# Illumina/Pisces

Measured on AMD Instinct MI355X. Metric: candidate loci/s at 500x depth, higher is better.
Workload: dtype int32 counts + f64 likelihoods; 1 GPU; BASELINE config 2: synthetic 100000 loci x 500x amplicon pileup, SNV-only, gVCF, per GPU per step; device-resident packed tuples; depth=500, ring_batches=6, tile_loci=56, parallelism=interval-shard x1

## Files before the change

### pisces_amd/csrc/device_math.hip.h

```cpp
#pragma once
#include <hip/hip_runtime.h>
#include <stdint.h>

#include "../../include/pisces_hip.h"
#include "poisson_core.h"

namespace pisces {

struct DeviceParams {
    int32_t min_bq, noise_level, max_vq, min_vq, vq_filter, min_cov, low_depth_filter;
    int32_t min_gq, max_gq, low_gq_filter, sb_model, filter_single_strand, include_ref, emit_zero_cov;
    int32_t rmxn_max_len, rmxn_min_rep;
    float min_freq, vf_filter, gt_min_freq, target_lod, nocall_thr, rmxn_freq_limit;
    double sb_threshold;
    double err_q;
    double err_sb;
    double ln10;
    unsigned long long* totals;
    const double* q_to_p_lut;
    int32_t q_to_p_n;
    const double* gq_tail;
    int32_t gq_tail_a, gq_tail_cov;
    int32_t refs_only;
    int32_t variants_only;
// ... 405 lines not shown
        reverseBias = (rev.var_gt_zero * fwd.false_pos) / overall.var_gt_zero;
        if (overall.var_gt_zero == 0) {
            forwardBias = 1;
            reverseBias = 1;
        }
    }
    double score = forwardBias > reverseBias ? forwardBias : reverseBias;
    cov_both = (cf > 0) && (cr > 0);
    var_both = (sf > 0) && (sr > 0);
    if (!cov_both) score = 0;
    bias_score = score;
    acceptable = score < P.sb_threshold;
    return ok0 && ok1 && ok2;
}

__device__ __forceinline__ int32_t somatic_gq_index(int32_t genotype, int32_t cov, int32_t support, const DeviceParams& P)
{
    if (cov == 0 || !((genotype == PISCES_GT_HOM_REF) || (genotype == PISCES_GT_HOM_ALT))) return -1;
    const float nonAlleleObservationsF = (1.0f - frequency_f(support, cov)) * (float)cov;
    const float expectedNonAllelObservationsF = P.target_lod * (float)cov;
    if (nonAlleleObservationsF >= expectedNonAllelObservationsF) return -1;
    const int ai = (int)((double)nonAlleleObservationsF + 1.0);
    if (ai >= 1 && ai < P.gq_tail_a && cov < P.gq_tail_cov) return ai * P.gq_tail_cov + cov;
    return -1;
}
__device__ __forceinline__ bool somatic_gq_try(int32_t genotype, int32_t variantQ, int32_t cov, int32_t support, const DeviceParams& P,
                                               int32_t gq_index, int32_t gq_cap_value , int32_t& gq)
{
    const bool noCall = (genotype == PISCES_GT_ALT12_LIKE_NOCALL || genotype == PISCES_GT_ALT_LIKE_NOCALL || genotype == PISCES_GT_REF_LIKE_NOCALL);
    if ((cov == 0) || noCall) { gq = P.min_gq; return true; }
    if ((genotype == PISCES_GT_HOM_REF) || (genotype == PISCES_GT_HOM_ALT)) {
        if (gq_index >= 0 && variantQ == P.max_vq && P.gq_cap) { gq = gq_cap_value; return true; }
        const float nonAlleleObservationsF = (1.0f - frequency_f(support, cov)) * (float)cov;
        const float expectedNonAllelObservationsF = P.target_lod * (float)cov;
        if (nonAlleleObservationsF >= expectedNonAllelObservationsF) { gq = P.min_gq; return true; }
        return false;
    }
    double qScore = fmin((double)P.max_gq, (double)variantQ);
    qScore = fmax(qScore, (double)P.min_gq);
    gq = (int32_t)rint(qScore);
    return true;
}

struct AlleleTables {
    int32_t vq;
    double sb[3];
    int32_t gq_cap;
    int32_t gq_idx;
    uint32_t have;
};
__device__ __forceinline__ bool tables_complete(const DeviceParams& P) { return P.vq_tab && P.sb_tab && P.sb0_tab && P.gq_cap; }

__device__ __forceinline__ AlleleTables request_allele_tables(bool isRef, int32_t support, int32_t total, int32_t refsup, const int32_t cov[3],
                                                              const int32_t sup[3], const DeviceParams& P)
{
    AlleleTables t;
    const uint32_t tab_cov = (uint32_t)P.tab_cov;
    const bool vq_in = support > 0 && total > 0 && support < P.vq_tab_k && total < P.tab_cov;
    const int16_t vq_v = P.vq_tab[vq_in ? (uint32_t)support * tab_cov + (uint32_t)total : 0u];
    const int s2 = sup[2] / 2, c2 = cov[2] / 2;
    const int ss[3] = {sup[0] + sup[1] + sup[2], sup[0] + s2, sup[1] + s2};
    const int cc[3] = {cov[0] + cov[1] + cov[2], cov[0] + c2, cov[1] + c2};
    double sb_v[3];
    uint32_t have = vq_in ? 1u : 0u;
#pragma unroll
    for (int w = 0; w < 3; w++) {
        const bool zero = ss[w] == 0;
        const bool in = zero ? (P.sb_model != PISCES_SB_POISSON && cc[w] >= 0 && cc[w] < P.tab_cov)
                             : (ss[w] > 0 && ss[w] < P.sb_tab_k && cc[w] >= 0 && cc[w] < P.tab_cov);
        const double* base = zero ? P.sb0_tab : P.sb_tab;
        const uint32_t idx = in ? (zero ? (uint32_t)cc[w] : (uint32_t)ss[w] * tab_cov + (uint32_t)cc[w]) : 0u;
        sb_v[w] = base[idx];
        have |= in ? (2u << w) : 0u;
    }
    t.gq_idx = somatic_gq_index(somatic_genotype(isRef, total, support, refsup, P), total, support, P);
    const int16_t gq_v = P.gq_cap[t.gq_idx >= 0 ? t.gq_idx : 0];
    t.vq = vq_v;
    t.sb[0] = sb_v[0]; t.sb[1] = sb_v[1]; t.sb[2] = sb_v[2];
    t.gq_cap = gq_v;
    t.have = have;
    return t;
}

__device__ __forceinline__ bool poisson_qscore_try(int32_t callCount, int32_t coverage, const DeviceParams& P, const AlleleTables& t, int32_t& vq)
{
    if ((callCount <= 0) || (coverage <= 0)) { vq = 0; return true; }
    if (t.have & 1u) { vq = t.vq; return true; }
    const double lambda = P.err_q * coverage;
    if (P.max_vq <= 110 && callCount >= 3 && (double)callCount >= 2.0 * lambda) {
        const double km1 = callCount - 1;
        const double need = ((double)P.max_vq + 1.0) * 0.23025850929940458 + 1e-3;
        if (km1 * (ln_ratio_lower_bound(km1, lambda) - 1.0) >= need) { vq = P.max_vq; return true; }
    }
    return false;
}

__device__ __forceinline__ bool sb_stats_try(int32_t support, int32_t coverage, const DeviceParams& P, bool have, double value, SbStats& st)
{
    st.support = (double)support;
    st.coverage = (double)coverage;
    if (support == 0) {
        if (P.sb_model == PISCES_SB_POISSON) {
            st.false_pos = 1;
            st.var_gt_zero = 0;
            return true;
        }
        if (!have) return false;
        st.var_gt_zero = value;
        st.false_pos = 1 - st.var_gt_zero;
        return true;
    }
    if (have) {
        st.var_gt_zero = value;
    } else {
        const double a = (double)support, x = (double)coverage * P.err_sb;
        if (!(x > 0.0 && 2.0 * x <= a && a * (ln_ratio_lower_bound(a, x) - 1.0) + x > 51.0)) return false;
        st.var_gt_zero = 1.0;
    }
    st.false_pos = fmax(0.0, 1 - st.var_gt_zero);
    return true;
}

__device__ __forceinline__ bool strand_bias_try(const int32_t cov[3], const int32_t sup[3], const DeviceParams& P, const AlleleTables& t,
                                                double& bias_score, int& acceptable, int& var_both, int& cov_both)
{
    const int s2 = sup[2] / 2, c2 = cov[2] / 2;
    const int sf = sup[0] + s2, sr = sup[1] + s2, cf = cov[0] + c2, cr = cov[1] + c2;
    SbStats overall, fwd, rev;
    const bool ok0 = sb_stats_try(sup[0] + sup[1] + sup[2], cov[0] + cov[1] + cov[2], P, (t.have & 2u) != 0, t.sb[0], overall);
    const bool ok1 = sb_stats_try(sf, cf, P, (t.have & 4u) != 0, t.sb[1], fwd);
    const bool ok2 = sb_stats_try(sr, cr, P, (t.have & 8u) != 0, t.sb[2], rev);
    double forwardBias = 0.0, reverseBias = 0.0;
    if (!(fwd.false_pos == 0.0 && rev.false_pos == 0.0 && overall.var_gt_zero > 0.0)) {
        forwardBias = (fwd.var_gt_zero * rev.false_pos) / overall.var_gt_zero;
        reverseBias = (rev.var_gt_zero * fwd.false_pos) / overall.var_gt_zero;
        if (overall.var_gt_zero == 0) {
            forwardBias = 1;
            reverseBias = 1;
        }
    }
    double score = forwardBias > reverseBias ? forwardBias : reverseBias;
    cov_both = (cf > 0) && (cr > 0);
    var_both = (sf > 0) && (sr > 0);
    if (!cov_both) score = 0;
    bias_score = score;
    acceptable = score < P.sb_threshold;
    return ok0 && ok1 && ok2;
}

__device__ __noinline__ int32_t poisson_qscore_out_of_line(int32_t callCount, int32_t coverage, double err, int32_t max_vq, double ln10)
{
    const QParams q = {max_vq, ln10};
    return poisson_qscore_core(callCount, coverage, err, q);
}
struct SbPair { double var_gt_zero, false_pos; };
__device__ __noinline__ SbPair sb_stats_out_of_line(double support, double coverage, double noiseFreq, int model)
{
    const SbStats st = sb_create_stats<false>(support, coverage, noiseFreq, 0.0, model);
    SbPair p = {st.var_gt_zero, st.false_pos};
    return p;
}
__device__ inline SbResult strand_bias_out_of_line(const int32_t cov[3], const int32_t sup[3], const DeviceParams& P)
{
    const int s2 = sup[2] / 2, c2 = cov[2] / 2;
    SbStats st[3];
#pragma unroll 1
// ... 66 lines not shown
```

### pisces_amd/csrc/kernels.hip.h

```cpp
#pragma once
#include <hip/hip_runtime.h>
#include <stdint.h>

#include "device_math.hip.h"
#include "genotype_core.h"

namespace pisces {

constexpr int kBlock = 256;
constexpr int kTile = 64;
constexpr int kFolded = 18;
constexpr int kUnroll = 8;
constexpr int kSlotsPerTile = 4 * kTile;
#ifndef PISCES_TOTAL_SHARDS
#define PISCES_TOTAL_SHARDS 64
#endif
constexpr int kTotalShards = PISCES_TOTAL_SHARDS;
constexpr int kTotalStride = 16;
constexpr int kRefMargin = 32;
constexpr int kRefWin = kTile + 2 * kRefMargin;
constexpr int kWaveRows = 32;
constexpr int kWaveRow = kTile;
constexpr int kWaveRegion = kWaveRows * kWaveRow;
constexpr int kQLutLds = 128;

typedef uint32_t u32x4 __attribute__((ext_vector_type(4)));

__device__ __forceinline__ int allele_of_rank(int k) { return k == 1 ? 2 : (k == 2 ? 1 : k); }
__device__ __forceinline__ int rank_of_allele(int a) { return a == 1 ? 2 : (a == 2 ? 1 : a); }

__device__ __forceinline__ int allele_type_of_base(uint8_t c)
{
    return c == 'A' ? 0 : c == 'G' ? 1 : c == 'C' ? 2 : c == 'T' ? 3 : 4;
}

__device__ __forceinline__ void accumulate_folded(int* hist, uint32_t t, uint32_t n_loci, uint32_t min_bq)
{
    uint32_t locus = PISCES_TUPLE_LOCUS(t);
    uint32_t dir = PISCES_TUPLE_DIR(t);
    uint32_t allele = PISCES_TUPLE_ALLELE(t);
    uint32_t qual = PISCES_TUPLE_QUAL(t);
    if (allele < 4u && qual < min_bq) allele = 4u;
    if (locus < n_loci && dir < 3u && allele < 6u) atomicAdd(&hist[(allele * 3u + dir) * kTile + locus], 1);
}

__device__ __forceinline__ void accumulate_wave(int* hist, uint32_t t, uint32_t min_bq_shifted)
{
    const uint32_t region = (t < min_bq_shifted) ? (uint32_t)(kWaveRegion * sizeof(int)) : 0u;
    const uint32_t off = (t & 0x1FFCu) | region;
    atomicAdd(reinterpret_cast<int*>(reinterpret_cast<char*>(hist) + off), 1);
}

template <typename Op>
__device__ __forceinline__ void stream_tuples(const uint32_t* __restrict__ tuples, int64_t begin, int64_t end, Op op)
{
    const int tid = threadIdx.x;
    int64_t abegin = (begin + 3) & ~(int64_t)3;
    int64_t aend = end & ~(int64_t)3;
    if (abegin > aend) { abegin = end; aend = end; }
    for (int64_t i = begin + tid; i < abegin; i += kBlock) op(tuples[i]);
    const u32x4* __restrict__ p4 = reinterpret_cast<const u32x4*>(tuples + abegin);
    const int64_t n4 = (aend - abegin) >> 2;
    for (int64_t i = tid; i < n4; i += (int64_t)kBlock * kUnroll) {
        u32x4 v[kUnroll];
#pragma unroll
        for (int u = 0; u < kUnroll; u++) {
            int64_t j = i + (int64_t)u * kBlock;
            v[u] = j < n4 ? __builtin_nontemporal_load(&p4[j]) : (u32x4){~0u, ~0u, ~0u, ~0u};
        }
#pragma unroll
        for (int u = 0; u < kUnroll; u++) {
            op(v[u].x); op(v[u].y); op(v[u].z); op(v[u].w);
        }
    }
    for (int64_t i = aend + tid; i < end; i += kBlock) op(tuples[i]);
}

__device__ __forceinline__ void copy_record(PiscesCalledAllele* dst, const PiscesCalledAllele* src)
{
    const unsigned long long sb = (unsigned long long)__double_as_longlong(src->strand_bias_score);
    uint4* dp = reinterpret_cast<uint4*>(dst);
    dp[0] = make_uint4((uint32_t)src->position, (uint32_t)src->total_coverage, (uint32_t)src->allele_support, (uint32_t)src->reference_support);
    dp[1] = make_uint4((uint32_t)src->num_no_calls, (uint32_t)src->coverage_by_dir[0], (uint32_t)src->coverage_by_dir[1], (uint32_t)src->coverage_by_dir[2]);
    dp[2] = make_uint4((uint32_t)src->support_by_dir[0], (uint32_t)src->support_by_dir[1], (uint32_t)src->support_by_dir[2], (uint32_t)src->variant_qscore);
    dp[3] = make_uint4((uint32_t)sb, (uint32_t)(sb >> 32), (uint32_t)(uint16_t)src->genotype_qscore | ((uint32_t)(uint16_t)src->noise_level << 16), (uint32_t)src->filter_bits | ((uint32_t)src->info << 16));
}

struct PointCounts {
    int cov[3], sup[3];
    int total, nocalls, refsup, support;
};

struct HistBlock {
    static __device__ __forceinline__ int idx(int a, int d, int l) { return (a * 3 + d) * kTile + l; }
};
struct HistWave {
    static __device__ __forceinline__ int idx(int a, int d, int l) { return (a * 4 + d) * kWaveRow + (int)PISCES_TUPLE_COLUMN(l, d); }
};

struct HistLinear {
    static __device__ __forceinline__ int idx(int a, int d, int l) { return (a * 4 + d) * kWaveRow + l; }
};

struct LocusCounts { int h[6][3]; };

template <typename H = HistBlock>
__device__ __forceinline__ LocusCounts load_counts(const int* hist, int l)
{
    LocusCounts lc;
#pragma unroll
    for (int k = 0; k < kFolded; k++) lc.h[k / 3][k % 3] = hist[H::idx(k / 3, k % 3, l)];
    return lc;
}

template <typename HistWave = pisces::HistWave>
__device__ __forceinline__ LocusCounts load_counts_wave(const int* hist, int l)
// ... 351 lines not shown
            v[u] = __builtin_nontemporal_load(&p4[j]);
        }
    };
    auto consume = [&](const u32x4* v) {
#pragma unroll
        for (int u = 0; u < kWaveUnroll; u++) { op(v[u].x); op(v[u].y); op(v[u].z); op(v[u].w); }
    };
    const bool streams = (uint32_t)wid < nb;
    if (NW == 2) {
        if (streams) load(cur, (uint32_t)__builtin_amdgcn_readfirstlane(wid));
        __builtin_amdgcn_sched_barrier(0);
        pre();
    } else {
        pre();
        if (streams) load(cur, (uint32_t)__builtin_amdgcn_readfirstlane(wid));
    }
    for (int64_t i = begin + tid; i < abegin; i += 64 * NW) op(tuples[i]);
    if (streams) {
        uint32_t b = (uint32_t)__builtin_amdgcn_readfirstlane(wid);
        const uint32_t m = (nb - b + NW - 1) / NW;
        for (uint32_t p = (m - 1) / 2; p > 0; p--) {
            load(nxt, b + NW);
            __builtin_amdgcn_sched_barrier(0);
            consume(cur);
            __builtin_amdgcn_sched_barrier(0);
            load(cur, b + 2 * NW);
            __builtin_amdgcn_sched_barrier(0);
            consume(nxt);
            __builtin_amdgcn_sched_barrier(0);
            b += 2 * NW;
        }
        if (((m - 1) & 1u) != 0) {
            load(nxt, b + NW);
            __builtin_amdgcn_sched_barrier(0);
            consume(cur);
            __builtin_amdgcn_sched_barrier(0);
#pragma unroll
            for (int u = 0; u < kWaveUnroll; u++) cur[u] = nxt[u];
            b += NW;
        }
        if (b == nb - 1 && (n4 % kBatch)) {
#pragma unroll
            for (int u = 0; u < kWaveUnroll; u++)
                if (b * kBatch + (uint32_t)u * 64u + (uint32_t)lane >= n4) cur[u] = (u32x4){~0u, ~0u, ~0u, ~0u};
        }
        consume(cur);
    }
    for (int64_t i = aend + tid; i < end; i += 64 * NW) op(tuples[i]);
}

__device__ __forceinline__ void wave_lds_sync()
{
    __builtin_amdgcn_fence(__ATOMIC_SEQ_CST, "workgroup");
    __builtin_amdgcn_wave_barrier();
}

template <typename H = HistWave>
__device__ __forceinline__ uint32_t slow_alleles(const int* hist, const uint8_t* s_refwin, uint32_t slow, int l, int pos, int rt, int ref_rank,
                                                 const uint8_t* __restrict__ ref, int64_t win_lo, int64_t win_hi, PiscesCalledAllele* slots,
                                                 const DeviceParams& P)
{
    uint32_t called = 0;
    const int ref_a = (rt < 4) ? rt : PISCES_ALLELE_N;
#pragma unroll 1
    for (int k = 0; k < 5; k++) {
        if (!((slow >> k) & 1u)) continue;
        const bool isRef = k == 4;
        const int a = isRef ? ref_a : allele_of_rank(k);
        const LocusCounts lc = load_counts_wave<H>(hist, l);
        const PointCounts c = point_counts_of(lc, a, isRef, rt, 0);
        int vq = 0;
        if (c.support > 0 && c.total != 0) vq = poisson_qscore_out_of_line(c.support, c.total, P.err_q, P.max_vq, P.ln10);
        if (!isRef && vq < P.min_vq) continue;
        SbResult sb = {0.0, 0, 0, 0};
        if (c.support > 0) sb = strand_bias_out_of_line(c.cov, c.sup, P);
        PiscesCalledAllele r;
        (void)finish_allele<false>(c, pos, a, isRef, rt, vq, sb, ref, win_lo, win_hi, P, r, s_refwin, kRefMargin + l);
        copy_record(&slots[isRef ? ref_rank : k], &r);
        if (!isRef) called |= 1u << k;
    }
    return called;
}

template <int NW, typename H = HistWave>
__device__ __forceinline__ void call_phase_wave(const int* hist, const uint8_t* s_refwin, uint8_t* s_vmask, const PiscesTile& tile, const int t,
                                                const int l, const int wid, const uint8_t* __restrict__ ref, const int32_t ref_start,
                                                const int64_t ref_len, PiscesCalledAllele* __restrict__ records,
                                                PiscesTileResult* __restrict__ tile_results, const DeviceParams& P
#ifdef PISCES_TIMING
                                                , const long long tc0, const long long tc1
#endif
                                                )
{
    const int pos = tile.start_position + l;
    const uint8_t refb = s_refwin[kRefMargin + l];
    const bool in_ref = l < tile.n_loci && refb != 0;
    const int rt = in_ref ? allele_type_of_base(refb) : PISCES_ALLELE_N;
    const int64_t win_lo = (int64_t)ref_start - 1, win_hi = win_lo + ref_len;
    auto slot_of = [&](int k) { return records + ((int64_t)t * kSlotsPerTile + l * 4 + k); };
    const bool dirty = locus_is_dirty(P, pos);
    const LocusCounts lc = load_counts_wave<H>(hist, l);
    const bool ref_wave = wid == 0, var_wave = wid == NW - 1;
    if (P.folded_out && ref_wave && l < tile.n_loci) {
        const unsigned rel = (unsigned)(pos - P.folded_first);
        if (rel < (unsigned)P.folded_n) {
            int32_t* const dst = P.folded_out + (size_t)rel * PISCES_FOLDED_PER_LOCUS;
#pragma unroll
            for (int a = 0; a < 6; a++)
#pragma unroll
                for (int d = 0; d < 3; d++) dst[a * 3 + d] = lc.h[a][d];
        }
    }

    const bool tabs = tables_complete(P);
    auto fast_allele = [&](const PointCounts& c, int a, bool isRef, PiscesCalledAllele& rec) -> bool {
        int vq = 0;
        double sb_score = 0.0;
        int sb_ok = 0, sb_var = 0, sb_cov = 0;
        if (!tabs) return false;
        const AlleleTables tb = request_allele_tables(isRef, c.support, c.total, c.refsup, c.cov, c.sup, P);
        if (c.support > 0 && c.total != 0 && !poisson_qscore_try(c.support, c.total, P, tb, vq)) return false;
        if (!isRef && vq < P.min_vq) return true;
        if (c.support > 0 && !strand_bias_try(c.cov, c.sup, P, tb, sb_score, sb_ok, sb_var, sb_cov)) return false;
        const GqPre g = {tb.gq_idx, tb.gq_cap};
        const SbResult sb = {sb_score, sb_ok, sb_var, sb_cov};
        if (!finish_allele<true>(c, pos, a, isRef, rt, vq, sb, ref, win_lo, win_hi, P, rec, s_refwin, kRefMargin + l, nullptr, &g)) return false;
        return true;
    };
    bool ref_emitted = false;
    int ref_rank = 0;
    uint32_t slow = 0;
    uint32_t vmask = 0;
    const int ref_a = (rt < 4) ? rt : PISCES_ALLELE_N;
    if (ref_wave) {
        const PointCounts c = point_counts_of(lc, ref_a, true, rt, 0);
        if (in_ref && P.include_ref && !P.variants_only && (P.emit_zero_cov || c.total + c.nocalls > 0)) {
            ref_rank = (rt < 4) ? rank_of_allele(rt) : 0;
            ref_emitted = true;
            PiscesCalledAllele rec;
            if (fast_allele(c, ref_a, true, rec)) copy_record(slot_of(ref_rank), &rec);
            else slow |= 16u;
        }
    }
#ifdef PISCES_TIMING
    const long long tcA = wall_clock64();
#endif
    if (var_wave && in_ref && rt < 4 && !P.refs_only && !dirty) {
#pragma unroll 1
        for (int k = 0; k < 4; k++) {
            const int a = allele_of_rank(k);
            if (a == rt) continue;
            const PointCounts c = point_counts_of(lc, a, false, rt, 0);
            if (c.support == 0) continue;
            if (!variant_passes_frequency(c, P)) continue;
            PiscesCalledAllele r;
            r.position = 0;
            if (!fast_allele(c, a, false, r)) { slow |= 1u << k; continue; }
            if (r.position == 0) continue;
            copy_record(slot_of(k), &r);
            vmask |= 1u << k;
        }
    }
    if (__builtin_expect(__ballot(slow != 0) != 0ull, 0))
        vmask |= slow_alleles<H>(hist, s_refwin, slow, l, pos, rt, ref_rank, ref, win_lo, win_hi, records + ((int64_t)t * kSlotsPerTile + l * 4), P);
    if (NW == 2) {
        if (var_wave) s_vmask[l] = (uint8_t)vmask;
        __syncthreads();
        if (!ref_wave) return;
        vmask = s_vmask[l];
    }
#ifdef PISCES_TIMING
    const long long tcB = wall_clock64();
#endif

    const uint32_t valid = vmask ? vmask : (ref_emitted ? (1u << ref_rank) : 0u);
    int n_surv = 0, n_var = 0;
#pragma unroll
    for (int k = 0; k < 4; k++) {
        n_surv += __popcll(__ballot((valid >> k) & 1u));
        n_var += __popcll(__ballot((vmask >> k) & 1u));
    }
    const int n_call_total = n_var + __popcll(__ballot(ref_emitted));
    const int n_loci_called = __popcll(__ballot(valid != 0));
    uint32_t word = valid << ((l & 7) * 4);
    word |= __shfl_xor(word, 1, 64);
    word |= __shfl_xor(word, 2, 64);
    word |= __shfl_xor(word, 4, 64);
    PiscesTileResult* const tile_result = &tile_results[t];
    if ((l & 7) == 0) tile_result->valid[l >> 3] = word;
    if (l == 0) {
        tile_result->record_begin = t * kSlotsPerTile;
        tile_result->n_records = n_surv;
        tile_result->n_candidate_loci = n_loci_called;
        tile_result->n_called = n_call_total;
        if (P.totals) {
            unsigned long long* tt = P.totals + (size_t)(t % kTotalShards) * kTotalStride;
            atomicAdd(&tt[0], (unsigned long long)n_surv);
            atomicAdd(&tt[1], (unsigned long long)n_loci_called);
            atomicAdd(&tt[2], (unsigned long long)n_call_total);
            atomicAdd(&tt[3], 1ull);
        }
#ifdef PISCES_TIMING
        const long long tc2 = wall_clock64();
        tile_result->record_begin = (int)(tc0 & 0x3FFFFFFF);
        tile_result->n_records = (int)(tc1 & 0x3FFFFFFF);
        tile_result->n_candidate_loci = (int)(tc2 & 0x3FFFFFFF);
        tile_result->n_called = (int)__builtin_amdgcn_s_getreg(63492);
        tile_result->valid[0] = __builtin_amdgcn_s_getreg(63508);
        tile_result->valid[1] = 0;
        tile_result->valid[2] = (uint32_t)(tcA - tc1);
        tile_result->valid[3] = (uint32_t)(tcB - tcA);
        tile_result->valid[4] = 0;
        tile_result->valid[5] = (uint32_t)(tc2 - tcB);
#endif
    }
}

template <int NW>
__global__ __launch_bounds__(64 * NW, NW == 1 ? PISCES_WAVE_OCC : PISCES_WAVE2_OCC) void call_tiles_wave_kernel(
    const uint32_t* __restrict__ tuples, const PiscesTile* __restrict__ tiles, int32_t n_tiles,
    const uint8_t* __restrict__ ref, int32_t ref_start, int64_t ref_len, PiscesCalledAllele* __restrict__ records,
    PiscesTileResult* __restrict__ tile_results, DeviceParams P, const DeviceParams* __restrict__ Pd )
{
    __shared__ __attribute__((aligned(16))) int hist[2 * kWaveRegion];
    __shared__ uint8_t s_refwin[kRefWin];
    __shared__ uint8_t s_vmask[kTile];

    const int t = blockIdx.x;
    if (t >= n_tiles) return;
    const int l = threadIdx.x & 63, wid = threadIdx.x >> 6;
    const PiscesTile tile = tiles[t];
#ifdef PISCES_TIMING
    const long long tc0 = wall_clock64();
#endif
    auto setup = [&]() {
        int4* h4 = reinterpret_cast<int4*>(hist);
        for (int i = threadIdx.x; i < 2 * kWaveRegion / 4; i += 64 * NW) h4[i] = make_int4(0, 0, 0, 0);
        for (int i = threadIdx.x; i < kRefWin; i += 64 * NW) {
            const int64_t ri = (int64_t)tile.start_position - kRefMargin + i - ref_start;
            s_refwin[i] = (ri >= 0 && ri < ref_len) ? ref[ri] : (uint8_t)0;
        }
        __syncthreads();
    };

    {
        if (NW == 2) __builtin_amdgcn_s_setprio(3);
        const uint32_t min_bq_shifted = (uint32_t)min(max(P.min_bq, 0), 255) << 24;
        stream_tuples_wave<NW>(tuples, tile.tuple_begin, tile.tuple_end, l, wid, [&](uint32_t v) { accumulate_wave(hist, v, min_bq_shifted); }, setup);
    }
    __syncthreads();
    if (NW == 2) __builtin_amdgcn_s_setprio(0);
#ifdef PISCES_TIMING
    const long long tc1 = wall_clock64();
#endif

    call_phase_wave<NW>(hist, s_refwin, s_vmask, tile, t, l, wid, ref, ref_start, ref_len, records, tile_results, P
#ifdef PISCES_TIMING
                        , tc0, tc1
#endif
                        );
}

__global__ __launch_bounds__(256) void build_vq_tab_kernel(int16_t* __restrict__ tab, int32_t n_k, int32_t n_cov, DeviceParams P)
{
    const int64_t i = (int64_t)blockIdx.x * blockDim.x + threadIdx.x;
    if (i >= (int64_t)n_k * n_cov) return;
    tab[i] = (int16_t)poisson_qscore((int32_t)(i / n_cov), (int32_t)(i % n_cov), P);
}
__global__ __launch_bounds__(256) void build_sb_tab_kernel(double* __restrict__ tab, double* __restrict__ tab0, int32_t n_k, int32_t n_cov, DeviceParams P)
{
    const int64_t i = (int64_t)blockIdx.x * blockDim.x + threadIdx.x;
    if (i >= (int64_t)n_k * n_cov) return;
    const int k = (int)(i / n_cov), cov = (int)(i % n_cov);
    tab[i] = k >= 1 ? fmax(0.0, poisson_cdf_sb((double)k - 1, (double)cov * P.err_sb)) : 0.0;
    if (k == 0) tab0[cov] = pow(1 - P.err_sb, (double)cov);
}
__global__ __launch_bounds__(256) void build_gq_cap_kernel(int16_t* __restrict__ tab, const double* __restrict__ gq_tail, int32_t n_a, int32_t n_cov, DeviceParams P)
{
    const int64_t i = (int64_t)blockIdx.x * blockDim.x + threadIdx.x;
    if (i >= (int64_t)n_a * n_cov) return;
    if (i < n_cov) { tab[i] = 0; return; }
    double rawQ = p_to_q(q_to_p_int(P.max_vq, P) + gq_tail[i]);
    double qScore = fmin((double)P.max_gq, rawQ);
    qScore = fmax(qScore, (double)P.min_gq);
    tab[i] = (int16_t)rint(qScore);
}

__global__ __launch_bounds__(64) void totals_collect_kernel(unsigned long long* __restrict__ shards, unsigned long long* __restrict__ out_host, int reset)
{
    const int l = threadIdx.x;
    if (l < 4) {
        unsigned long long v = 0;
        for (int sh = 0; sh < kTotalShards; sh++) v += shards[sh * kTotalStride + l];
        out_host[l] = v;
    }
    if (reset)
        for (int i = l; i < kTotalShards * kTotalStride; i += 64) shards[i] = 0ull;
    __threadfence_system();
}

__global__ __launch_bounds__(256) void read_probe_kernel(const u32x4* __restrict__ p, int64_t n4, uint32_t* __restrict__ sink)
{
    uint32_t acc = 0;
    const int64_t stride = (int64_t)gridDim.x * blockDim.x * 8;
    for (int64_t i = (int64_t)blockIdx.x * blockDim.x * 8 + threadIdx.x; i < n4; i += stride) {
        u32x4 v[8];
#pragma unroll
        for (int u = 0; u < 8; u++) {
            const int64_t j = i + (int64_t)u * blockDim.x;
            v[u] = j < n4 ? __builtin_nontemporal_load(&p[j]) : (u32x4){0u, 0u, 0u, 0u};
        }
#pragma unroll
        for (int u = 0; u < 8; u++) acc ^= v[u].x ^ v[u].y ^ v[u].z ^ v[u].w;
    }
    if (acc == 0x9E3779B9u) *sink = acc;
}

__global__ __launch_bounds__(256) void read_probe_dword_kernel(const uint32_t* __restrict__ p, int64_t n, uint32_t* __restrict__ sink)
{
    uint32_t acc = 0;
    const int64_t stride = (int64_t)gridDim.x * blockDim.x * 8;
    for (int64_t i = (int64_t)blockIdx.x * blockDim.x * 8 + threadIdx.x; i < n; i += stride) {
        uint32_t v[8];
#pragma unroll
        for (int u = 0; u < 8; u++) {
            const int64_t j = i + (int64_t)u * blockDim.x;
            v[u] = j < n ? p[j] : 0u;
        }
#pragma unroll
        for (int u = 0; u < 8; u++) acc ^= v[u];
    }
    if (acc == 0x9E3779B9u) *sink = acc;
}

__global__ void build_gq_tail_kernel(double* __restrict__ table, int32_t n_a, int32_t n_cov, float target_lod)
{
    const int64_t i = (int64_t)blockIdx.x * blockDim.x + threadIdx.x;
    if (i >= (int64_t)n_a * n_cov) return;
    const int a = (int)(i / n_cov), cov = (int)(i % n_cov);
// ... 770 lines not shown
```

### pisces_amd/csrc/store_kernels.hip.h

```cpp
#pragma once
#include <hip/hip_runtime.h>
#include <stdint.h>
#include <type_traits>

#include "kernels.hip.h"
#include "read_walk.h"
#include "stream_kernels.hip.h"

#ifndef PISCES_ADD_OCC
#define PISCES_ADD_OCC 6
#endif
#ifdef PISCES_ADD_STAMPS
#define PISCES_STAMP(k, is_max) do { if (threadIdx.x == 0) A.stamps[(long long)blockIdx.x * 8 + ((k) == 0 ? 2 : (k) == 1 ? 3 : (k) - 2)] = (long long)wall_clock64(); } while (0)
#else
#define PISCES_STAMP(k, is_max) do { } while (0)
#endif
namespace pisces {

struct ReadDesc {
    int32_t pos0;
    uint32_t meta;
    int64_t aoff;
};
struct ReadExt {
// ... 1218 lines not shown
    tile.n_loci = min(step, R.block_size - i * step);
    tile.tuple_begin = tile.tuple_end = 0;
    return tile;
}

__device__ __forceinline__ int xcd_tile_of_block(int b, int n)
{
    const int x = b & 7, j = b >> 3, q = n >> 3, rem = n & 7;
    return x * q + min(x, rem) + j;
}

__device__ __forceinline__ int exchanged_tile(const StoreView& S, const PiscesTile* __restrict__ tiles, const RegularTiles& R, int n_tiles, int cus, int b, int lane,
                                          int* pre_lo , int* pre_hi)
{
    *pre_lo = -1;
    *pre_hi = 0;
    const int x = b & 7, j = b >> 3, q = n_tiles >> 3, rem = n_tiles & 7;
    const int first = x * q + min(x, rem), cnt = q + (x < rem ? 1 : 0), own = first + j;
    const int s = cnt / cus, r = cnt - s * cus, k = j / cus, c = j - k * cus;
    if (k >= s || S.n_segments < 1) return own;
    int g, grp, m;
    if (r > 0) {
        g = min(cus / r, 8);
        if (g < 2) return own;
        if (c < r) { grp = c; m = 0; }
        else { const int d = c - r; grp = d / (g - 1); m = 1 + d - grp * (g - 1); if (grp >= r) return own; }
    } else {
        g = 4; grp = c >> 2; m = c & 3;
        if (grp * 4 + 4 > cus) return own;
    }
    const SegmentView& G = S.seg[0];
    if (G.n_frags <= 0 || G.state[kStateUnsorted] != 0 || !G.grid || (G.state[kStateFrags] & kGridBadBit)) return own;
    const int reach = G.state[kStateReach];
    const int i = lane & 31;
    int a = 0, t_i = own;
    if (i < g) {
        const int c_i = r > 0 ? (i == 0 ? grp : r + grp * (g - 1) + i - 1) : grp * 4 + i;
        t_i = first + k * cus + c_i;
        const int start = tiles ? tiles[t_i].start_position : regular_tile(R, t_i).start_position;
        const int tile_end = start + kTile - 1;
        const int xq = (lane >> 5) ? (tile_end == 0x7FFFFFFF ? 0x7FFFFFFF : tile_end + 1) : (int)max((long long)start - reach + 1, -0x7FFFFFFFll);
        const long long kk = (long long)max(xq, 0) - G.grid_base;
        a = kk < 0 ? 0 : G.n_frags;
        if (kk >= 0 && kk < G.grid_n) a = min(G.grid[kk], G.n_frags);
    }
    const int cost = __shfl_down(a, 32) - a;
    int rank = 0;
    for (int u = 0; u < g; u++) {
        const int cu = __builtin_amdgcn_readlane(cost, u);
        rank += (cu < cost || (cu == cost && u < i)) ? 1 : 0;
    }
    const int want = r > 0 ? (m == 0 ? 0 : 1 + (m - 1 + k) % (g - 1)) : (m + k) & 3;
    const unsigned long long hit = __ballot(lane < g && rank == want);
    if (hit == 0ull) return own;
    const int chosen = (int)__ffsll((long long)hit) - 1;
    *pre_lo = __builtin_amdgcn_readlane(a, chosen);
    *pre_hi = __builtin_amdgcn_readlane(a, chosen + 32);
    return __builtin_amdgcn_readlane(t_i, chosen);
}

__device__ __forceinline__ uint32_t allele_row_bytes(uint32_t c)
{
    return (c == 'A' ? (uint32_t)PISCES_ALLELE_A : c == 'C' ? (uint32_t)PISCES_ALLELE_C : c == 'G' ? (uint32_t)PISCES_ALLELE_G
            : c == 'T' ? (uint32_t)PISCES_ALLELE_T : (uint32_t)PISCES_ALLELE_N) * (4u * kWaveRow * (uint32_t)sizeof(int));
}

__device__ __forceinline__ uint32_t allele_row_bytes_of_base(uint32_t c)
{
    const uint32_t t8 = (c << 2) & 0x18u;
    const uint32_t letter = (0x47544341u >> t8) & 0xFFu;
    const uint32_t code = (0x01030200u >> t8) & 0xFFu;
    return (c == letter ? code : (uint32_t)PISCES_ALLELE_N) * (4u * kWaveRow * (uint32_t)sizeof(int));
}

template <int NW>
__global__ __launch_bounds__(64 * NW, NW == 1 ? PISCES_WAVE_OCC : PISCES_WAVE2_OCC) void call_store_tiles_kernel(
    StoreView S, const uint32_t* __restrict__ tuples, const PiscesTile* __restrict__ tiles , RegularTiles R, int32_t n_tiles,
    int32_t trade_cus , int32_t walk_prio, const uint8_t* __restrict__ ref, int32_t ref_start, int64_t ref_len, PiscesCalledAllele* __restrict__ records,
    PiscesTileResult* __restrict__ tile_results, DeviceParams P, const DeviceParams* __restrict__ Pd)
{
    __shared__ __attribute__((aligned(16))) int hist[2 * kWaveRegion];
    __shared__ uint8_t s_refwin[kRefWin];
    __shared__ uint8_t s_vmask[kTile];
    __shared__ unsigned long long s_masktab[kMaskTab];
    __shared__ uint2 s_pairs[NW][kPairSlots];

    if ((int)blockIdx.x >= n_tiles) return;
    int pre_lo = -1, pre_hi = 0;
    const int t = trade_cus > 0 ? exchanged_tile(S, tiles, R, n_tiles, trade_cus, (int)blockIdx.x, (int)(threadIdx.x & 63), &pre_lo, &pre_hi)
                                : xcd_tile_of_block((int)blockIdx.x, n_tiles);
    const int l = threadIdx.x & 63, wid = __builtin_amdgcn_readfirstlane((int)(threadIdx.x >> 6));
    const PiscesTile tile = tiles ? tiles[t] : regular_tile(R, t);
#ifdef PISCES_STORE_TIMING
    const long long tc0 = wall_clock64();
    long long stamps[6] = {0, 0, 0, 0, 0, 0};
#endif
    {
        int4* h4 = reinterpret_cast<int4*>(hist);
        for (int i = threadIdx.x; i < 2 * kWaveRegion / 4; i += 64 * NW) h4[i] = make_int4(0, 0, 0, 0);
        for (int i = threadIdx.x; i < kRefWin; i += 64 * NW) {
            const int64_t ri = (int64_t)tile.start_position - kRefMargin + i - ref_start;
            s_refwin[i] = (ri >= 0 && ri < ref_len) ? ref[ri] : (uint8_t)0;
        }
        for (int i = threadIdx.x; i < kMaskTab; i += 64 * NW) {
            const int a = i / 9, e = i - 9 * a;
            const unsigned long long ge_a = a >= 8 ? 0ull : ~0ull << (8 * a), ge_e = e >= 8 ? 0ull : ~0ull << (8 * e);
            s_masktab[i] = ge_a & ~ge_e;
        }
        __syncthreads();
    }
    if (walk_prio) __builtin_amdgcn_s_setprio(3);
    const uint32_t min_bq = (uint32_t)min(max(P.min_bq, 0), 127);
    char* const hbytes = reinterpret_cast<char*>(hist);
    constexpr uint32_t kRegionBytes = (uint32_t)(kWaveRegion * sizeof(int));
    for (int64_t i = tile.tuple_begin + threadIdx.x; i < tile.tuple_end; i += 64 * NW) {
        const uint32_t v = tuples[i];
        const uint32_t dir = PISCES_TUPLE_DIR(v), allele = PISCES_TUPLE_ALLELE(v);
        if (dir < 3u && allele < 6u)
            atomicAdd(reinterpret_cast<int*>(hbytes + ((PISCES_TUPLE_QUAL(v) < min_bq) ? kRegionBytes : 0u) +
                                             (uint32_t)HistLinear::idx((int)allele, (int)dir, (int)PISCES_TUPLE_LOCUS(v)) * (uint32_t)sizeof(int)), 1);
    }
    auto on_obs = [&](int position, uint32_t allele, uint32_t dir, int, uint32_t qual) {
        const uint32_t off = ((qual < min_bq) ? kRegionBytes : 0u) +
                             (uint32_t)HistLinear::idx((int)allele, (int)dir, position - tile.start_position) * (uint32_t)sizeof(int);
        atomicAdd(reinterpret_cast<int*>(hbytes + off), 1);
    };
    for (int sg = 0; sg < S.n_segments; sg++) {
        const SegmentView& G = S.seg[sg];
#ifdef PISCES_STORE_TIMING
        if (G.dirs) walk_segment_fast<true>(G, tile.start_position, min_bq, l, wid, NW, hbytes, s_masktab, s_pairs[wid], on_obs, sg == 0 ? pre_lo : -1, pre_hi, stamps);
        else walk_segment_fast<false>(G, tile.start_position, min_bq, l, wid, NW, hbytes, s_masktab, s_pairs[wid], on_obs, sg == 0 ? pre_lo : -1, pre_hi, stamps);
#else
        if (G.dirs) walk_segment_fast<true>(G, tile.start_position, min_bq, l, wid, NW, hbytes, s_masktab, s_pairs[wid], on_obs, sg == 0 ? pre_lo : -1, pre_hi);
        else walk_segment_fast<false>(G, tile.start_position, min_bq, l, wid, NW, hbytes, s_masktab, s_pairs[wid], on_obs, sg == 0 ? pre_lo : -1, pre_hi);
#endif
    }
#ifdef PISCES_STORE_TIMING
    const long long tc_walk = wall_clock64();
#endif
    __syncthreads();
    if (NW > 2 && wid != 0 && wid != NW - 1) return;
    if (walk_prio) __builtin_amdgcn_s_setprio(0);
    call_phase_wave<(NW == 1 ? 1 : 2), HistLinear>(hist, s_refwin, s_vmask, tile, t, l, NW == 1 ? 0 : (wid == NW - 1 ? 1 : 0), ref, ref_start, ref_len, records, tile_results, P
#ifdef PISCES_TIMING
                                    , 0ll, 0ll
#endif
                                    );
#ifdef PISCES_STORE_TIMING
    if (threadIdx.x == 0) {
        const long long tc_end = wall_clock64();
        int* tr = reinterpret_cast<int*>(&records[(int64_t)t * kSlotsPerTile + kSlotsPerTile - 1]);
        tr[0] = (int)(tc0 & 0x3FFFFFFF);
        tr[1] = (int)(stamps[0] & 0x3FFFFFFF);
        tr[2] = (int)(tc_walk & 0x3FFFFFFF);
        tr[3] = (int)(tc_end & 0x3FFFFFFF);
        tr[4] = (int)stamps[1];
        tr[7] = (int)stamps[2]; tr[8] = (int)stamps[3]; tr[9] = (int)stamps[4]; tr[10] = (int)stamps[5];
        tr[5] = (int)__builtin_amdgcn_s_getreg(63492);
        tr[6] = (int)__builtin_amdgcn_s_getreg(63508);
        tr[11] = (int)blockIdx.x;
    }
#endif
}

__global__ __launch_bounds__(64) void compact_small_kernel(const PiscesCalledAllele* __restrict__ records, const PiscesTileResult* __restrict__ tr,
                                                           int32_t n_tiles, PiscesCalledAllele* __restrict__ out, int32_t capacity)
{
    const int l = threadIdx.x, t = blockIdx.x;
    const int v = l < n_tiles ? tr[l].n_records : 0;
    int incl = v;
#pragma unroll
    for (int d = 1; d < 64; d <<= 1) {
        const int y = __shfl_up(incl, d, 64);
        if (l >= d) incl += y;
    }
    const int my_off = __shfl(incl - v, t, 64);
    if (t == 0) {
        int called = l < n_tiles ? tr[l].n_called : 0;
#pragma unroll
        for (int d = 32; d >= 1; d >>= 1) called += __shfl_xor(called, d, 64);
        if (l == 63) reinterpret_cast<int4*>(out)[0] = make_int4(incl, called, 0, 0);
    }
    const uint32_t nib = (tr[t].valid[l >> 3] >> ((l & 7) * 4)) & 0xFu;
    int x = __popc(nib);
    const int mine = x;
#pragma unroll
    for (int d = 1; d < 64; d <<= 1) {
        const int y = __shfl_up(x, d, 64);
        if (l >= d) x += y;
    }
    int64_t dst = (int64_t)my_off + (x - mine);
    const PiscesCalledAllele* src = records + (int64_t)tr[t].record_begin + l * 4;
    for (int k = 0; k < 4; k++) {
        if (!(nib & (1u << k))) continue;
        if (dst < capacity) copy_record(&out[1 + dst], &src[k]);
        dst++;
    }
}

__global__ __launch_bounds__(1024) void accumulate_store_tiles_kernel(StoreView S, const uint32_t* __restrict__ tuples, const PiscesTile* __restrict__ tiles,
                                                                        int32_t n_tiles, int32_t* __restrict__ counts, int32_t min_bq_,
                                                                        unsigned long long* __restrict__ sumq, const ulonglong2* __restrict__ bq_lut)
{
    __shared__ int hist[kTile * kAnchStride];
    const int t = blockIdx.x;
    if (t >= n_tiles) return;
    const PiscesTile tile = tiles[t];
    for (int i = threadIdx.x; i < kTile * kAnchStride; i += (int)blockDim.x) hist[i] = 0;
    __syncthreads();
    const uint32_t n_loci = (uint32_t)tile.n_loci, min_bq = (uint32_t)min_bq_;
    auto add = [&](uint32_t locus, uint32_t allele, uint32_t dir, uint32_t anchor, uint32_t qual) {
        if (allele < 4u && qual < min_bq) allele = 4u;
        if (locus < n_loci && dir < 3u && allele < 6u && anchor < (uint32_t)PISCES_NUM_ANCHORS) {
            atomicAdd(&hist[locus * kAnchStride + (allele * 3u + dir) * PISCES_NUM_ANCHORS + anchor], 1);
            if (sumq && allele < 4u) {
                const ulonglong2 q = bq_lut[qual];
                unsigned long long* cell = &sumq[2 * (((int64_t)t * kTile + locus) * PISCES_COUNTS_PER_LOCUS + (allele * 3u + dir) * PISCES_NUM_ANCHORS + anchor)];
                atomicAdd(cell, q.x);
                atomicAdd(cell + 1, q.y);
            }
        }
    };
    const int sub = (int)blockIdx.y, n_sub = (int)gridDim.y;
    for (int64_t i = tile.tuple_begin + (int64_t)sub * blockDim.x + threadIdx.x; i < tile.tuple_end; i += (int64_t)blockDim.x * n_sub) {
        const uint32_t v = tuples[i];
        add(PISCES_TUPLE_LOCUS(v), PISCES_TUPLE_ALLELE(v), PISCES_TUPLE_DIR(v), PISCES_TUPLE_ANCHOR(v), v >> 24);
// ... 25 lines not shown
```

Before: 2.565 billion candidate loci/s.

## Split reference-allele calling across waves with LDS strand-bias handover

```diff
diff --git a/pisces_amd/csrc/device_math.hip.h b/pisces_amd/csrc/device_math.hip.h
--- a/pisces_amd/csrc/device_math.hip.h
+++ b/pisces_amd/csrc/device_math.hip.h
@@ -511,6 +511,44 @@
     return t;
 }
 
+__device__ __forceinline__ AlleleTables request_qscore_tables(bool isRef, int32_t support, int32_t total, int32_t refsup, const DeviceParams& P)
+{
+    AlleleTables t;
+    const bool vq_in = support > 0 && total > 0 && support < P.vq_tab_k && total < P.tab_cov;
+    const int16_t vq_v = P.vq_tab[vq_in ? (uint32_t)support * (uint32_t)P.tab_cov + (uint32_t)total : 0u];
+    t.gq_idx = somatic_gq_index(somatic_genotype(isRef, total, support, refsup, P), total, support, P);
+    const int16_t gq_v = P.gq_cap[t.gq_idx >= 0 ? t.gq_idx : 0];
+    t.vq = vq_v;
+    t.sb[0] = 0.0; t.sb[1] = 0.0; t.sb[2] = 0.0;
+    t.gq_cap = gq_v;
+    t.have = vq_in ? 1u : 0u;
+    return t;
+}
+__device__ __forceinline__ AlleleTables request_strand_tables(const int32_t cov[3], const int32_t sup[3], const DeviceParams& P)
+{
+    AlleleTables t;
+    const uint32_t tab_cov = (uint32_t)P.tab_cov;
+    const int s2 = sup[2] / 2, c2 = cov[2] / 2;
+    const int ss[3] = {sup[0] + sup[1] + sup[2], sup[0] + s2, sup[1] + s2};
+    const int cc[3] = {cov[0] + cov[1] + cov[2], cov[0] + c2, cov[1] + c2};
+    uint32_t have = 0u;
+#pragma unroll
+    for (int w = 0; w < 3; w++) {
+        const bool zero = ss[w] == 0;
+        const bool in = zero ? (P.sb_model != PISCES_SB_POISSON && cc[w] >= 0 && cc[w] < P.tab_cov)
+                             : (ss[w] > 0 && ss[w] < P.sb_tab_k && cc[w] >= 0 && cc[w] < P.tab_cov);
+        const double* base = zero ? P.sb0_tab : P.sb_tab;
+        const uint32_t idx = in ? (zero ? (uint32_t)cc[w] : (uint32_t)ss[w] * tab_cov + (uint32_t)cc[w]) : 0u;
+        t.sb[w] = base[idx];
+        have |= in ? (2u << w) : 0u;
+    }
+    t.vq = 0;
+    t.gq_cap = 0;
+    t.gq_idx = -1;
+    t.have = have;
+    return t;
+}
+
 __device__ __forceinline__ bool poisson_qscore_try(int32_t callCount, int32_t coverage, const DeviceParams& P, const AlleleTables& t, int32_t& vq)
 {
     if ((callCount <= 0) || (coverage <= 0)) { vq = 0; return true; }
diff --git a/pisces_amd/csrc/kernels.hip.h b/pisces_amd/csrc/kernels.hip.h
--- a/pisces_amd/csrc/kernels.hip.h
+++ b/pisces_amd/csrc/kernels.hip.h
@@ -31,7 +31,10 @@
 
 __device__ __forceinline__ int allele_type_of_base(uint8_t c)
 {
-    return c == 'A' ? 0 : c == 'G' ? 1 : c == 'C' ? 2 : c == 'T' ? 3 : 4;
+    const uint32_t t8 = ((uint32_t)c << 2) & 0x18u;
+    const uint32_t letter = (0x47544341u >> t8) & 0xFFu;
+    const uint32_t code = (0x01030200u >> t8) & 0xFFu;
+    return (uint32_t)c == letter ? (int)code : 4;
 }
 
 __device__ __forceinline__ void accumulate_folded(int* hist, uint32_t t, uint32_t n_loci, uint32_t min_bq)
@@ -549,8 +552,50 @@
     return called;
 }
 
+struct SbHandover {
+    double score;
+    uint32_t bits;
+    uint32_t pad;
+};
+constexpr uint32_t kSbMissed = 8u;
+
+enum : uint32_t {
+    kUniTabs = 1u,
+    kUniRefOn = 2u,
+    kUniZeroCov = 4u,
+    kUniVarsOn = 8u,
+    kUniDirty = 16u,
+    kUniFolded = 32u,
+};
+__device__ __forceinline__ uint32_t launch_predicates(const DeviceParams& P)
+{
+    const uint32_t u = (tables_complete(P) ? kUniTabs : 0u) | ((P.include_ref && !P.variants_only) ? kUniRefOn : 0u) |
+                       (P.emit_zero_cov ? kUniZeroCov : 0u) | (!P.refs_only ? kUniVarsOn : 0u) | (P.dirty_bits ? kUniDirty : 0u) |
+                       (P.folded_out ? kUniFolded : 0u);
+    return (uint32_t)__builtin_amdgcn_readfirstlane((int)u);
+}
+
+typedef const __attribute__((address_space(4))) char* KernargBytes;
+__device__ __forceinline__ DeviceParams reload_params(uint32_t kernarg_offset )
+{
+    KernargBytes p = (KernargBytes)__builtin_amdgcn_kernarg_segment_ptr() + kernarg_offset;
+    asm volatile("" : "+s"(p));
+    DeviceParams P;
+    __builtin_memcpy(&P, (const __attribute__((address_space(4))) DeviceParams*)p, sizeof(P));
+    return P;
+}
+
+__device__ __forceinline__ void store_record_head(PiscesCalledAllele* dst, const PiscesCalledAllele& r)
+{
+    uint4* dp = reinterpret_cast<uint4*>(dst);
+    dp[0] = make_uint4((uint32_t)r.position, (uint32_t)r.total_coverage, (uint32_t)r.allele_support, (uint32_t)r.reference_support);
+    dp[1] = make_uint4((uint32_t)r.num_no_calls, (uint32_t)r.coverage_by_dir[0], (uint32_t)r.coverage_by_dir[1], (uint32_t)r.coverage_by_dir[2]);
+    dp[2] = make_uint4((uint32_t)r.support_by_dir[0], (uint32_t)r.support_by_dir[1], (uint32_t)r.support_by_dir[2], (uint32_t)r.variant_qscore);
+}
+
 template <int NW, typename H = HistWave>
-__device__ __forceinline__ void call_phase_wave(const int* hist, const uint8_t* s_refwin, uint8_t* s_vmask, const PiscesTile& tile, const int t,
+__device__ __forceinline__ void call_phase_wave(const int* hist, const uint8_t* s_refwin, uint8_t* s_vmask, SbHandover* s_sb ,
+                                                const uint32_t uni , const PiscesTile& tile, const int t,
                                                 const int l, const int wid, const uint8_t* __restrict__ ref, const int32_t ref_start,
                                                 const int64_t ref_len, PiscesCalledAllele* __restrict__ records,
                                                 PiscesTileResult* __restrict__ tile_results, const DeviceParams& P
@@ -565,10 +610,17 @@
     const int rt = in_ref ? allele_type_of_base(refb) : PISCES_ALLELE_N;
     const int64_t win_lo = (int64_t)ref_start - 1, win_hi = win_lo + ref_len;
     auto slot_of = [&](int k) { return records + ((int64_t)t * kSlotsPerTile + l * 4 + k); };
-    const bool dirty = locus_is_dirty(P, pos);
+    const bool ref_wave = wid == 0, var_wave = wid == NW - 1;
+    uint32_t dirty_word = 0u, dirty_rel = 0u;
+    bool dirty_in = false;
+    if ((uni & kUniDirty) && var_wave) {
+        dirty_rel = (unsigned)(pos - P.dirty_first);
+        dirty_in = dirty_rel < (unsigned)P.dirty_n;
+        dirty_word = P.dirty_bits[dirty_in ? (dirty_rel >> 5) : 0u];
+    }
     const LocusCounts lc = load_counts_wave<H>(hist, l);
-    const bool ref_wave = wid == 0, var_wave = wid == NW - 1;
-    if (P.folded_out && ref_wave && l < tile.n_loci) {
+    const bool dirty = dirty_in && ((dirty_word >> (dirty_rel & 31u)) & 1u) != 0u;
+    if ((uni & kUniFolded) && ref_wave && l < tile.n_loci) {
         const unsigned rel = (unsigned)(pos - P.folded_first);
         if (rel < (unsigned)P.folded_n) {
             int32_t* const dst = P.folded_out + (size_t)rel * PISCES_FOLDED_PER_LOCUS;
@@ -579,7 +631,7 @@
         }
     }
 
-    const bool tabs = tables_complete(P);
+    const bool tabs = (uni & kUniTabs) != 0u;
     auto fast_allele = [&](const PointCounts& c, int a, bool isRef, PiscesCalledAllele& rec) -> bool {
         int vq = 0;
         double sb_score = 0.0;
@@ -599,20 +651,41 @@
     uint32_t slow = 0;
     uint32_t vmask = 0;
     const int ref_a = (rt < 4) ? rt : PISCES_ALLELE_N;
-    if (ref_wave) {
+    uint32_t ref_w3z = 0u, ref_w3w = 0u;
+    bool ref_q_ok = false;
+    if (NW == 1) {
         const PointCounts c = point_counts_of(lc, ref_a, true, rt, 0);
-        if (in_ref && P.include_ref && !P.variants_only && (P.emit_zero_cov || c.total + c.nocalls > 0)) {
+        if (in_ref && (uni & kUniRefOn) && ((uni & kUniZeroCov) || c.total + c.nocalls > 0)) {
             ref_rank = (rt < 4) ? rank_of_allele(rt) : 0;
             ref_emitted = true;
             PiscesCalledAllele rec;
             if (fast_allele(c, ref_a, true, rec)) copy_record(slot_of(ref_rank), &rec);
             else slow |= 16u;
         }
+    } else {
+        const PointCounts c = point_counts_of(lc, ref_a, true, rt, 0);
+        ref_emitted = in_ref && (uni & kUniRefOn) && ((uni & kUniZeroCov) || c.total + c.nocalls > 0);
+        ref_rank = (ref_emitted && rt < 4) ? rank_of_allele(rt) : 0;
+        if (ref_wave && tabs) {
+            const AlleleTables tb = request_qscore_tables(true, c.support, c.total, c.refsup, P);
+            int vq = 0;
+            const bool vq_ok = !(c.support > 0 && c.total != 0) || poisson_qscore_try(c.support, c.total, P, tb, vq);
+            const GqPre g = {tb.gq_idx, tb.gq_cap};
+            const SbResult no_sb = {0.0, 0, 0, 0};
+            PiscesCalledAllele rec;
+            const bool fin_ok = finish_allele<true>(c, pos, ref_a, true, rt, vq, no_sb, ref, win_lo, win_hi, P, rec, s_refwin, kRefMargin + l, nullptr, &g);
+            ref_q_ok = vq_ok && fin_ok;
+            if (ref_emitted && ref_q_ok) {
+                store_record_head(slot_of(ref_rank), rec);
+                ref_w3z = (uint32_t)(uint16_t)rec.genotype_qscore | ((uint32_t)(uint16_t)rec.noise_level << 16);
+                ref_w3w = (uint32_t)rec.filter_bits | ((uint32_t)rec.info << 16);
+            }
+        }
     }
 #ifdef PISCES_TIMING
     const long long tcA = wall_clock64();
 #endif
-    if (var_wave && in_ref && rt < 4 && !P.refs_only && !dirty) {
+    if (var_wave && in_ref && rt < 4 && (uni & kUniVarsOn) && !dirty) {
 #pragma unroll 1
         for (int k = 0; k < 4; k++) {
             const int a = allele_of_rank(k);
@@ -628,6 +701,22 @@
             vmask |= 1u << k;
         }
     }
+    if (NW == 2 && var_wave) {
+        const PointCounts c = point_counts_of(lc, ref_a, true, rt, 0);
+        SbHandover ho = {0.0, 0u, 0u};
+        if (tabs) {
+            const AlleleTables tb = request_strand_tables(c.cov, c.sup, P);
+            double sb_score = 0.0;
+            int sb_ok = 0, sb_var = 0, sb_cov = 0;
+            const bool hit = strand_bias_try(c.cov, c.sup, P, tb, sb_score, sb_ok, sb_var, sb_cov);
+            const bool has = c.support > 0;
+            ho.score = has ? sb_score : 0.0;
+            ho.bits = has ? ((uint32_t)sb_ok | ((uint32_t)sb_var << 1) | ((uint32_t)sb_cov << 2) | (hit ? 0u : kSbMissed)) : 0u;
+        } else {
+            ho.bits = kSbMissed;
+        }
+        s_sb[l] = ho;
+    }
     if (__builtin_expect(__ballot(slow != 0) != 0ull, 0))
         vmask |= slow_alleles<H>(hist, s_refwin, slow, l, pos, rt, ref_rank, ref, win_lo, win_hi, records + ((int64_t)t * kSlotsPerTile + l * 4), P);
     if (NW == 2) {
@@ -635,6 +724,14 @@
         __syncthreads();
         if (!ref_wave) return;
         vmask = s_vmask[l];
+        const SbHandover ho = s_sb[l];
+        const bool ref_slow = ref_emitted && (!ref_q_ok || (ho.bits & kSbMissed) != 0u);
+        if (ref_emitted && !ref_slow) {
+            const unsigned long long sb = (unsigned long long)__double_as_longlong(ho.score);
+            reinterpret_cast<uint4*>(slot_of(ref_rank))[3] = make_uint4((uint32_t)sb, (uint32_t)(sb >> 32), ref_w3z, ref_w3w | ((ho.bits & 7u) << 29));
+        }
+        if (__builtin_expect(__ballot(ref_slow) != 0ull, 0))
+            (void)slow_alleles<H>(hist, s_refwin, ref_slow ? 16u : 0u, l, pos, rt, ref_rank, ref, win_lo, win_hi, records + ((int64_t)t * kSlotsPerTile + l * 4), P);
     }
 #ifdef PISCES_TIMING
     const long long tcB = wall_clock64();
@@ -683,6 +780,11 @@
     }
 }
 
+struct WaveKernelArgs {
+    const uint32_t* tuples; const PiscesTile* tiles; int32_t n_tiles; const uint8_t* ref; int32_t ref_start; int64_t ref_len;
+    PiscesCalledAllele* records; PiscesTileResult* tile_results; DeviceParams P; const DeviceParams* Pd;
+};
+
 template <int NW>
 __global__ __launch_bounds__(64 * NW, NW == 1 ? PISCES_WAVE_OCC : PISCES_WAVE2_OCC) void call_tiles_wave_kernel(
     const uint32_t* __restrict__ tuples, const PiscesTile* __restrict__ tiles, int32_t n_tiles,
@@ -692,11 +794,13 @@
     __shared__ __attribute__((aligned(16))) int hist[2 * kWaveRegion];
     __shared__ uint8_t s_refwin[kRefWin];
     __shared__ uint8_t s_vmask[kTile];
+    __shared__ SbHandover s_sb[NW == 1 ? 1 : kTile];
 
     const int t = blockIdx.x;
     if (t >= n_tiles) return;
     const int l = threadIdx.x & 63, wid = threadIdx.x >> 6;
     const PiscesTile tile = tiles[t];
+    const uint32_t uni = launch_predicates(P);
 #ifdef PISCES_TIMING
     const long long tc0 = wall_clock64();
 #endif
@@ -721,7 +825,8 @@
     const long long tc1 = wall_clock64();
 #endif
 
-    call_phase_wave<NW>(hist, s_refwin, s_vmask, tile, t, l, wid, ref, ref_start, ref_len, records, tile_results, P
+    const DeviceParams Pc = reload_params((uint32_t)offsetof(WaveKernelArgs, P));
+    call_phase_wave<NW>(hist, s_refwin, s_vmask, s_sb, uni, tile, t, l, wid, ref, ref_start, ref_len, records, tile_results, Pc
 #ifdef PISCES_TIMING
                         , tc0, tc1
 #endif
diff --git a/pisces_amd/csrc/store_kernels.hip.h b/pisces_amd/csrc/store_kernels.hip.h
--- a/pisces_amd/csrc/store_kernels.hip.h
+++ b/pisces_amd/csrc/store_kernels.hip.h
@@ -1324,6 +1324,7 @@
     __shared__ __attribute__((aligned(16))) int hist[2 * kWaveRegion];
     __shared__ uint8_t s_refwin[kRefWin];
     __shared__ uint8_t s_vmask[kTile];
+    __shared__ SbHandover s_sb[NW == 1 ? 1 : kTile];
     __shared__ unsigned long long s_masktab[kMaskTab];
     __shared__ uint2 s_pairs[NW][kPairSlots];
 
@@ -1383,7 +1384,7 @@
     __syncthreads();
     if (NW > 2 && wid != 0 && wid != NW - 1) return;
     if (walk_prio) __builtin_amdgcn_s_setprio(0);
-    call_phase_wave<(NW == 1 ? 1 : 2), HistLinear>(hist, s_refwin, s_vmask, tile, t, l, NW == 1 ? 0 : (wid == NW - 1 ? 1 : 0), ref, ref_start, ref_len, records, tile_results, P
+    call_phase_wave<(NW == 1 ? 1 : 2), HistLinear>(hist, s_refwin, s_vmask, s_sb, launch_predicates(P), tile, t, l, NW == 1 ? 0 : (wid == NW - 1 ? 1 : 0), ref, ref_start, ref_len, records, tile_results, P
 #ifdef PISCES_TIMING
                                     , 0ll, 0ll
 #endif
```

New measurement: 2.533 billion candidate loci/s. 0.987x the previous value.
